# skhu101/TDNN-F_NAS

Hardware: AMD Instinct MI355X
Metric: LF-MMI training frames/sec per node (SWBD 7q TDNN-F) (higher is better)
Workload: dtype f32

## Files before the change

### tdnn-f_nas_amd/csrc/abi_tdnn.hip

```cpp
#include <dlfcn.h>
#include <stdlib.h>
#include <string.h>

#include <string>

#include "common.h"
#include "gemm_f32.h"
#include "planes_gemm.h"

namespace tdnnf {

static thread_local std::string g_last_error;

void set_error(const char *fmt, ...) {
  char buf[1024];
  va_list ap;
  va_start(ap, fmt);
  vsnprintf(buf, sizeof(buf), fmt, ap);
  va_end(ap);
  g_last_error = buf;
}
int hip_status(hipError_t e, const char *what) {
  set_error("HIP error %d (%s) in %s", (int)e, hipGetErrorString(e), what);
  return TDNNF_EHIP;
}

Options &options() {
  static Options o;
  return o;
}

namespace {
typedef int (*roctx_push_t)(const char *);
typedef int (*roctx_pop_t)();
roctx_push_t g_roctx_push = nullptr;
roctx_pop_t g_roctx_pop = nullptr;
bool roctx_ready() {
  static const bool ok = [] {
    const char *e = getenv("TDNNF_ROCTX");
    if (e && atoi(e) == 0) return false;
    for (const char *lib : {"librocprofiler-sdk-roctx.so", "librocprofiler-sdk-roctx.so.1", "libroctx64.so", "libroctx64.so.4"}) {
      void *h = dlopen(lib, RTLD_NOW | RTLD_GLOBAL);
      if (!h) continue;
      g_roctx_push = (roctx_push_t)dlsym(h, "roctxRangePushA");
      g_roctx_pop = (roctx_pop_t)dlsym(h, "roctxRangePop");
      if (g_roctx_push && g_roctx_pop) return true;
    }
    return false;
  }();
  return ok;
}
}
TraceRange::TraceRange(const char *name) : on(roctx_ready()) {
  if (on) g_roctx_push(name);
}
TraceRange::~TraceRange() {
  if (on) g_roctx_pop();
}

bool tdnn_rows_ok(const tdnnf_tdnn_indexes *ix, int rows_in, int N) {
  if (!ix || ix->num_offsets < 1 || ix->num_offsets > TDNNF_MAX_OFFSETS || ix->row_stride < 1) return false;
  for (int i = 0; i < ix->num_offsets; i++) {
    const long long need = (long long)ix->row_offsets[i] + (long long)ix->row_stride * N - (ix->row_stride - 1);
    if (ix->row_offsets[i] < 0 || (N > 0 && rows_in < need)) return false;
  }
  return true;
}

}

using namespace tdnnf;

extern "C" {

const char *tdnnf_last_error(void) { return g_last_error.c_str(); }
int tdnnf_abi_version(void) { return 1; }

static int *option_slot(const char *name) {
  Options &o = options();
  if (!name) return nullptr;
  const struct { const char *n; int *p; } table[] = {{"ng_grouped", &o.ng_grouped}, {"ng_fuse", &o.ng_fuse}, {"ng_early_in", &o.ng_early_in},
                                                     {"wgrad_stream", &o.wgrad_stream}, {"gemm_ring", &o.gemm_ring}, {"planes", &o.planes}, {"den_split", &o.den_split}, {"phase_events", &o.phase_events}, {"wgrad_lag", &o.wgrad_lag}, {"ng_bk", &o.ng_bk}, {"ng_valu", &o.ng_valu}, {"ng_pform", &o.ng_pform}, {"planes_group", &o.planes_group}, {"xent_behind_den", &o.xent_behind_den}, {"ng_early_fork", &o.ng_early_fork}, {"ng_diag_skip", &o.ng_diag_skip}, {"wgrad_small", &o.wgrad_small}, {"splitk_per_cu", &o.splitk_per_cu}, {"gemm_alt_taps", &o.gemm_alt_taps}, {"reverse_passes", &o.reverse_passes}, {"splitk_partial_round", &o.splitk_partial_round}, {"wgrad_on_caller", &o.wgrad_on_caller}, {"den_mw_test_abort", &o.den_mw_test_abort}, {"planes_check_bound", &o.planes_check_bound}, {"den_gamma_pairs", &o.den_gamma_pairs}, {"num_form", &o.num_form}, {"align_form", &o.align_form}, {"align_checkpoint", &o.align_checkpoint}, {"align_path_checkpoint", &o.align_path_checkpoint}, {"num_frontier_cap", &o.num_frontier_cap}, {"gemm_arith_test", &o.gemm_arith_test}};
  for (auto &e : table)
    if (strcmp(e.n, name) == 0) return e.p;
  return nullptr;
}
int tdnnf_set_option(const char *name, int value) {
  int *p = option_slot(name);
  TDNNF_REQUIRE(p, "set_option: unknown option '%s' (ng_grouped, ng_fuse, ng_early_in, wgrad_stream, gemm_ring, planes, den_split, align_checkpoint, align_path_checkpoint)", name ? name : "(null)");
  *p = value;
  return TDNNF_OK;
}
int tdnnf_get_option(const char *name, int *value) {
  int *p = option_slot(name);
  TDNNF_REQUIRE(p && value, "get_option: unknown option '%s'", name ? name : "(null)");
  *value = *p;
  return TDNNF_OK;
}

}

namespace tdnnf {
int tdnn_propagate_impl(const tdnnf_tdnn_indexes *ix, const tdnnf_mat *in, const float *W, int ldw, int Do, int Di,
                        const float *bias, const float *eff_coef, int init_mode, int relu, tdnnf_mat *out, tdnnf_stream stream,
                        float *colstats, int *colstats_rows) {
  TDNNF_REQUIRE(mat_ok(in) && mat_ok(out) && W, "tdnn_propagate: bad matrices");
  TDNNF_REQUIRE(Do > 0 && Di > 0 && in->cols == Di && out->cols == Do, "tdnn_propagate: dims: in.cols=%d Di=%d out.cols=%d Do=%d",
                in ? in->cols : -1, Di, out ? out->cols : -1, Do);
  TDNNF_REQUIRE(tdnn_rows_ok(ix, in->rows, out->rows), "tdnn_propagate: input has too few rows for the time offsets");
  TDNNF_REQUIRE(ldw >= ix->num_offsets * Di, "tdnn_propagate: ldw < K*Di");
  TDNNF_REQUIRE(init_mode >= 0 && init_mode <= 2 && (init_mode != 1 || bias), "tdnn_propagate: init_mode 1 needs a bias");
  RowsGemmArgs a;
  memset(&a, 0, sizeof(a));
  a.A = in->data;
  a.lda = (long long)in->stride * ix->row_stride;
  a.B = W;
  a.ldb = ldw;
  a.C = out->data;
  a.ldc = out->stride;
  a.M = out->rows;
  a.N = Do;
  a.bias = bias;
  a.coef = eff_coef;
  a.init_mode = init_mode;
  a.relu = relu;
  a.colstats = colstats;
  a.colstats_rows = colstats_rows;
  a.nseg = ix->num_offsets;
  for (int i = 0; i < a.nseg; i++) {
    a.seg[i].a_off = (long long)ix->row_offsets[i] * in->stride;
    a.seg[i].b_off = (long long)i * Di;
    a.seg[i].klen = Di;
    a.seg[i].m_lo = 0;
    a.seg[i].m_hi = out->rows;
  }
  TDNNF_HIP(rows_gemm(a, true, (hipStream_t)stream));
  return TDNNF_OK;
}
}

extern "C" {

int tdnnf_tdnn_propagate(const tdnnf_tdnn_indexes *ix, const tdnnf_mat *in, const float *W, int ldw, int Do, int Di,
                         const float *bias, const float *eff_coef, int init_mode, tdnnf_mat *out, tdnnf_stream stream) {
  return tdnn_propagate_impl(ix, in, W, ldw, Do, Di, bias, eff_coef, init_mode, 0, out, stream);
}

}

namespace tdnnf {
int tdnn_backprop_data_impl(const tdnnf_tdnn_indexes *ix, const tdnnf_mat *out_deriv, const float *W, int ldw, int Do,
                            int Di, const float *eff_coef, int overwrite, const tdnnf_mat *add, float add_scale, int add_lo,
                            tdnnf_mat *in_deriv, tdnnf_stream stream) {
  TDNNF_REQUIRE(mat_ok(in_deriv) && mat_ok(out_deriv) && W, "tdnn_backprop_data: bad matrices");
  TDNNF_REQUIRE(Do > 0 && Di > 0 && in_deriv->cols == Di && out_deriv->cols == Do, "tdnn_backprop_data: bad dims");
  TDNNF_REQUIRE(tdnn_rows_ok(ix, in_deriv->rows, out_deriv->rows), "tdnn_backprop_data: in_deriv has too few rows for the time offsets");
  TDNNF_REQUIRE(ldw >= ix->num_offsets * Di, "tdnn_backprop_data: ldw < K*Di");
  const int rho = ix->row_stride, N = out_deriv->rows, K = ix->num_offsets;
  if (N == 0) return TDNNF_OK;
  for (int cls = 0; cls < rho; cls++) {
    RowsGemmArgs a;
    memset(&a, 0, sizeof(a));
    float cf_dummy = 0;
    (void)cf_dummy;
    int nseg = 0, u_max = 0;
// ... 171 lines not shown
```

### tdnn-f_nas_amd/csrc/common.h

```cpp
#pragma once
#include <hip/hip_runtime.h>
#include <stdarg.h>
#include <stdio.h>

#include "tdnnf_hip.h"

namespace tdnnf {

struct MatView {
  float *data;
  int rows, cols, stride;
};
inline MatView view(const tdnnf_mat *m) { return MatView{m->data, m->rows, m->cols, m->stride}; }

void set_error(const char *fmt, ...);
int hip_status(hipError_t e, const char *what);

inline bool mat_ok(const tdnnf_mat *m) {
  return m && m->rows >= 0 && m->cols >= 0 && m->stride >= m->cols && (m->data || m->rows * m->cols == 0);
}
inline bool same_dim(const tdnnf_mat *a, const tdnnf_mat *b) { return a->rows == b->rows && a->cols == b->cols; }

inline bool vec4_ok(const MatView &m) {
  return (reinterpret_cast<uintptr_t>(m.data) & 15) == 0 && m.stride % 4 == 0 && m.cols % 4 == 0;
}

#define TDNNF_REQUIRE(cond, ...)            \
  do {                                      \
    if (!(cond)) {                          \
      ::tdnnf::set_error(__VA_ARGS__);      \
      return TDNNF_EINVAL;                  \
    }                                       \
  } while (0)

#define TDNNF_HIP(expr)                                         \
  do {                                                          \
    hipError_t e__ = (expr);                                    \
    if (e__ != hipSuccess) return ::tdnnf::hip_status(e__, #expr); \
  } while (0)

#define TDNNF_LAUNCH_CHECK() TDNNF_HIP(hipGetLastError())

struct Options {
  int ng_grouped = 1;
  int ng_fuse = 1;
  int ng_early_in = 1;
  int wgrad_stream = -1;
  int gemm_ring = 1;
  int planes = 1;
  int den_mw_test_abort = 0;
  int planes_group = 1;
  int planes_check_bound = 0;
  int wgrad_lag = 3;
  int wgrad_on_caller = 0;
  int splitk_partial_round = 1;
  int reverse_passes = 0;
  int gemm_alt_taps = 1;
  int splitk_per_cu = 2;
  int wgrad_small = 0;
  int ng_bk = 0;
  int ng_early_fork = 1;
  int xent_behind_den = -1;
  int ng_pform = 1;
  int ng_valu = 0;
  int ng_diag_skip = 0;
  int phase_events = 0;
  int den_split = -1;
  int num_form = 0;
  int gemm_arith_test = 0;
  int num_frontier_cap = 0;
  int align_form = 0;
  int align_checkpoint = 0;
  int align_path_checkpoint = 0;
  int den_gamma_pairs = 0;
};
Options &options();

struct TraceRange {
  explicit TraceRange(const char *name);
  ~TraceRange();
  bool on;
};

__host__ __device__ inline float floor_keep_nan(float x, float f) { return x < f ? f : x; }

inline int grid_for(long long work, int block, int cap = 2048) {
  long long g = (work + block - 1) / block;
  if (g > cap) g = cap;
  if (g < 1) g = 1;
  return (int)g;
}
#ifdef __HIPCC__
template <class T>
struct as_given { typedef T type; };
template <class... P>
__attribute__((visibility("hidden"))) inline hipError_t launch_vec_or_scalar(bool vec, int rows, int cols, void (*k4)(P...), void (*k1)(P...), hipStream_t s, typename as_given<P>::type... args) {
  const long long work = (long long)rows * (vec ? cols / 4 : cols);
  void (*k)(P...) = vec ? k4 : k1;
  hipLaunchKernelGGL(k, dim3(grid_for(work, 256)), dim3(256), 0, s, args...);
  return hipGetLastError();
}
#endif

inline unsigned long long tdnnf_decision(unsigned long long step, unsigned long long k) {
  unsigned long long z = step * 0x9E3779B97F4A7C15ULL + k * 0xBF58476D1CE4E5B9ULL + 0x94D049BB133111EBULL;
  z = (z ^ (z >> 30)) * 0xBF58476D1CE4E5B9ULL;
  z = (z ^ (z >> 27)) * 0x94D049BB133111EBULL;
  return (z ^ (z >> 31)) >> 8;
}

bool log_softmax_propagate_with_aux(const tdnnf_mat *in, tdnnf_mat *out, tdnnf_mat *aux, float aux_scale, hipStream_t s);
float chain_supervision_weight(const tdnnf_supervision *sp);
size_t chain_split_region_bytes(const tdnnf_den_graph *g, int B, int T);
int chain_den(const tdnnf_den_graph *g, const tdnnf_supervision *sp, const tdnnf_mat *y, float leaky, tdnnf_mat *deriv, void *ws, hipStream_t s,
              bool beside_other_work = false, hipStream_t caller_aux = nullptr, hipEvent_t ev_recursions = nullptr, bool *ev_recorded = nullptr);
int chain_num_recursion(const tdnnf_supervision *sp, const tdnnf_den_graph *g, const tdnnf_mat *y, void *ws, hipStream_t s);
int chain_num_xent(const tdnnf_den_graph *g, const tdnnf_supervision *sp, const tdnnf_mat *y, const tdnnf_mat *xent_output, float xent_regularize,
                   tdnnf_mat *xent_deriv, void *ws, hipStream_t s, bool xent_deriv_initialised = false);
int chain_num(const tdnnf_den_graph *g, const tdnnf_supervision *sp, const tdnnf_mat *y, const tdnnf_mat *xent_output,
              float xent_regularize, tdnnf_mat *xent_deriv, void *ws, hipStream_t s, bool xent_deriv_initialised = false);
int chain_finish(const tdnnf_den_graph *g, const tdnnf_supervision *sp, const tdnnf_mat *y, float l2_regularize, double *results,
                 tdnnf_mat *deriv, tdnnf_mat *xent_deriv, void *ws, hipStream_t s);
int chain_objf_den(const tdnnf_den_graph *g, const tdnnf_supervision *sp, const tdnnf_mat *y, float leaky, void *ws, hipStream_t s);
int chain_objf_num_recursion(const tdnnf_supervision *sp, const tdnnf_den_graph *g, const tdnnf_mat *y, void *ws, hipStream_t s);
int chain_objf_num_xent(const tdnnf_den_graph *g, const tdnnf_supervision *sp, const tdnnf_mat *y, const tdnnf_mat *xent_output, void *ws, hipStream_t s);
int chain_objf_finish(const tdnnf_den_graph *g, const tdnnf_supervision *sp, const tdnnf_mat *y, float l2_regularize, double *results, void *ws, hipStream_t s);

bool tdnn_rows_ok(const tdnnf_tdnn_indexes *ix, int rows_in, int N);
int tdnn_propagate_impl(const tdnnf_tdnn_indexes *ix, const tdnnf_mat *in, const float *W, int ldw, int Do, int Di,
                        const float *bias, const float *eff_coef, int init_mode, int relu, tdnnf_mat *out, tdnnf_stream stream,
                        float *colstats = nullptr, int *colstats_rows = nullptr);
int tdnn_update_simple_impl(const tdnnf_tdnn_indexes *ix, const tdnnf_mat *in_value, const tdnnf_mat *out_deriv, int Do, int Di,
                            const float *eff_coef, float lr, float *W_acc, int ldw, float *bias_acc, void *ws, size_t ws_bytes,
                            const int *active_dev, int max_active, tdnnf_stream stream, bool overwrite = false);
int tdnn_backprop_data_impl(const tdnnf_tdnn_indexes *ix, const tdnnf_mat *out_deriv, const float *W, int ldw, int Do, int Di,
                            const float *eff_coef, int overwrite, const tdnnf_mat *add, float add_scale, int add_lo,
                            tdnnf_mat *in_deriv, tdnnf_stream stream);

}
// ... 1 lines not shown
```

### tdnn-f_nas_amd/csrc/fused.hip

```cpp
#include <algorithm>

#include "batchnorm.h"
#include "device.h"
#include "ew_dev.h"
#include "fused.h"
#include "gemm_f32.h"
#include "launch_forms.h"
#include "planes_gemm.h"

namespace tdnnf {
namespace {

__device__ __forceinline__ void store_planes4(const PlanesSink &pk, float ps, long long ra, int c, const float (&v)[4]) {
  typedef _Float16 h4 __attribute__((ext_vector_type(4)));
  h4 hi, lo;
#pragma unroll
  for (int j = 0; j < 4; j++) {
    const float w = v[j] * ps;
    hi[j] = (_Float16)w;
    lo[j] = (_Float16)(w - (float)hi[j]);
  }
  const int kb = c >> 4, k = c & 15, half = (k >> 3) ^ (int)((ra >> 3) & 1);
  _Float16 *dst = reinterpret_cast<_Float16 *>(pk.P) + (((long long)kb * 2) * pk.R + ra) * 16 + half * 8 + (k & 7);
  *reinterpret_cast<h4 *>(dst) = hi;
  *reinterpret_cast<h4 *>(dst + pk.R * 16) = lo;
}

template <int VEC, bool PLANES>
__global__ __launch_bounds__(256) void bn_apply_bypass_kernel(MatView x, const float *mean, const float *scale, int D, int period,
                                                              MatView prev, float bypass, MatView out, const float *mask, int B, PlanesSink pk, int rev) {
  const int cv = x.cols / VEC;
  const float ps = PLANES ? pk.rec[0] : 1.0f;
  const int ncb = PLANES ? cv / 8 : 1;
  const long long total = PLANES ? (long long)((x.rows + 7) / 8) * 8 * cv : (long long)x.rows * cv;
  for (long long e0 = blockIdx.x * 256LL + threadIdx.x; e0 < total; e0 += gridDim.x * 256LL) {
    const long long e = rev ? total - 1 - e0 : e0;
    int r, c;
    if (PLANES) {
      const long long blk = e >> 6;
      r = (int)(blk / ncb) * 8 + (int)((e >> 3) & 7);
      c = ((int)(blk % ncb) * 8 + (int)(e & 7)) * VEC;
      if (r >= x.rows) continue;
    } else {
      r = (int)(e / cv);
      c = (int)(e % cv) * VEC;
    }
    const int cd = c % period;
    if (cd >= D) continue;
    float xv[4], pv[4] = {0, 0, 0, 0}, o[4];
    ld(x.data + (long long)r * x.stride + c, xv, VEC == 4);
    if (prev.data) ld(prev.data + (long long)r * prev.stride + c, pv, VEC == 4);
    const float *mk = mask ? mask + (long long)(x.cols > D ? c / period : r % B) * D + cd : nullptr;
    float mu[4], sc[4], mv[4] = {1.f, 1.f, 1.f, 1.f};
    ld(mean + cd, mu, VEC == 4);
    ld(scale + cd, sc, VEC == 4);
    if (mk) ld(mk, mv, VEC == 4);
#pragma unroll
    for (int j = 0; j < VEC; j++) o[j] = (xv[j] - mu[j]) * sc[j] * mv[j] + bypass * pv[j];
    st(out.data + (long long)r * out.stride + c, o, VEC == 4);
    if constexpr (PLANES && VEC == 4) store_planes4(pk, ps, r, c, o);
  }
}

template <int VEC, bool RELU_STATS>
__global__ __launch_bounds__(256) void bn_relu_bwd_reduce_kernel(MatView x, MatView dz, const float *mean, const float *scale,
                                                                 int rows_per_chunk, int chunks, float *partial, const float *mask, int B) {
  __shared__ float red[5][4][64 * 4 + 4];
  const int tc = threadIdx.x & 63, tr = threadIdx.x >> 6;
  const int col = (blockIdx.x * 64 + tc) * VEC;
  const int r0 = blockIdx.y * rows_per_chunk, r1 = min(x.rows, r0 + rows_per_chunk);
  float s[5][4] = {};
  if (col < x.cols) {
    float mu[4], sc[4];
#pragma unroll
    for (int j = 0; j < VEC; j++) {
      mu[j] = mean[col + j];
      sc[j] = scale[col + j];
    }
    for (int r = r0 + tr; r < r1; r += 4) {
      float xv[4], dv[4];
      ld(x.data + (long long)r * x.stride + col, xv, VEC == 4);
      ld(dz.data + (long long)r * dz.stride + col, dv, VEC == 4);
      if (mask) {
        const float *mk = mask + (long long)(r % B) * x.cols + col;
#pragma unroll
        for (int j = 0; j < VEC; j++) dv[j] *= mk[j];
      }
#pragma unroll
      for (int j = 0; j < VEC; j++) {
        const float z = (xv[j] - mu[j]) * sc[j];
        s[0][j] += z * dv[j];
        s[1][j] += dv[j];
        s[2][j] += dv[j] * dv[j];
        if (RELU_STATS) {
          s[3][j] += xv[j];
          s[4][j] += xv[j] > 0.f ? 1.f : 0.f;
        }
      }
    }
  }
  constexpr int NQ = RELU_STATS ? 5 : 3;
#pragma unroll
  for (int q = 0; q < NQ; q++)
#pragma unroll
    for (int j = 0; j < VEC; j++) red[q][tr][tc * VEC + j] = s[q][j];
  __syncthreads();
  if (tr == 0 && col < x.cols) {
#pragma unroll
    for (int q = 0; q < NQ; q++)
#pragma unroll
      for (int j = 0; j < VEC; j++) {
        const int k = tc * VEC + j;
        partial[((long long)q * chunks + blockIdx.y) * x.cols + col + j] = (red[q][0][k] + red[q][1][k]) + (red[q][2][k] + red[q][3][k]);
      }
  }
}

__global__ __launch_bounds__(kFinThreads) void bn_relu_bwd_finalize_kernel(const float *partial, int chunks, int D, int N, float target_rms,
                                                                           float *memo, double *relu_stats, int test_mode, double *oderiv,
                                                                           double *sums_out = nullptr, const double *sums_in = nullptr, int N_local = 0,
                                                                           double *fro2 = nullptr, float repair_abs = 0.f) {
  __shared__ double red[5 * kFinLanes * (kFinCols + 1)];
  const int d = blockIdx.x * kFinCols + (threadIdx.x & (kFinCols - 1));
  double q[5];
  const int nq = relu_stats ? 5 : 3;
  if (!sums_in) finalize_sums<5, double>(partial, chunks, chunks, D, nq, q, red);
  if (sums_out) {
    if (threadIdx.x < kFinCols && d < D)
      for (int k = 0; k < nq; k++) sums_out[(size_t)k * D + d] = q[k];
    return;
  }
  if (relu_stats && blockIdx.x == 0 && threadIdx.x == 0) relu_stats[0] += (double)(sums_in ? N_local : N);
  if (oderiv && blockIdx.x == 0 && threadIdx.x == 0) oderiv[0] += (double)N;
  double bound = 0;
  if (threadIdx.x < kFinCols && d < D) {
    if (sums_in)
      for (int k = 0; k < nq; k++) q[k] = sums_in[(size_t)k * D + d];
    const float coeff = -1.0f / (target_rms * target_rms * N);
    const float sc = memo[2 * D + d];
    const float vdm = test_mode ? 0.f : (float)(coeff * q[0]) * sc;
    memo[3 * D + d] = vdm;
    memo[4 * D + d] = test_mode ? 0.f : (float)(-q[1] / N);
    if (relu_stats) {
      relu_stats[1 + d] += q[3];
      relu_stats[1 + D + d] += q[4];
    }
    if (oderiv || fro2) {
      const double sc2 = (double)sc * sc;
      double v = sc2 * (test_mode ? q[2] : q[2] - q[1] * q[1] / N);
      if (!test_mode) {
        const double var = (double)memo[D + d] - (double)memo[d] * memo[d];
        v += 2.0 * vdm * sc * q[0] + (double)vdm * vdm * (double)N * (var > 0 ? var : 0.0) * sc2;
      }
      if (oderiv) oderiv[1 + d] += v > 0 ? v : 0.0;
      const double nr = sqrt(v > 0 ? v : 0.0) * 1.0001 + sqrt((double)N) * repair_abs;
      bound = nr * nr;
    }
  }
  if (fro2 && threadIdx.x < 64) {
    for (int o = 16; o > 0; o >>= 1) bound += __shfl_xor(bound, o, 32);
    if (threadIdx.x == 0) fro2[blockIdx.x] = bound;
  }
}

template <int VEC, bool PLANES>
__global__ __launch_bounds__(256) void bn_relu_bwd_apply_kernel(MatView x, MatView dz, const float *memo, int D,
                                                                const double *repair_stats, float self_repair_scale,
                                                                int rows_per_chunk, int chunks, MatView d_aff, float *partial, const float *mask, int B,
                                                                PlanesSink pk, int pk_lead, int rev) {
  const float pks = PLANES ? pk.rec[0] : 1.0f;
  __shared__ float red[4][64 * 4 + 4];
  const int tc = threadIdx.x & 63, tr = threadIdx.x >> 6;
  const int col = (blockIdx.x * 64 + tc) * VEC;
  const int chunk = rev ? (int)gridDim.y - 1 - (int)blockIdx.y : (int)blockIdx.y;
  const int r0 = chunk * rows_per_chunk, r1 = min(x.rows, r0 + rows_per_chunk);
  float s[4] = {0, 0, 0, 0};
  if (col < x.cols) {
    float mu[4], sc[4], vdm[4], tmp[4], rep[4];
#pragma unroll
    for (int j = 0; j < VEC; j++) {
      mu[j] = memo[col + j];
// ... 156 lines not shown
      const int idx = t + 256 * j, n = idx >> 3, kk = (idx & 7) * 4;
      *reinterpret_cast<float4 *>(Bs + n * LD + kk) = wv[j];
    }
    if (k0 + BK < D) request(k0 + BK);
#pragma unroll
    for (int i = 0; i < 4; i++) {
      const int r = r0 + rr + 32 * i;
      if (FULL || r < x.rows) {
        st(d_aff.data + (long long)r * d_aff.stride + col, o[i], true);
        if constexpr (PLANES) store_planes4(pk, pks, (long long)pk_lead + r, col, o[i]);
      }
    }
#pragma unroll
    for (int j = 0; j < 4; j++) {
      float v = cs[j];
      v += __shfl_xor(v, 8, 64);
      v += __shfl_xor(v, 16, 64);
      v += __shfl_xor(v, 32, 64);
      if (lane < 8) colred[wave][lane * 4 + j] = v;
    }
    __syncthreads();
    {
      const float *as = As + (wave * 32 + li) * LD + lh * 4;
      const float *bs = Bs + li * LD + lh * 4;
#pragma unroll
      for (int kg = 0; kg < BK / 8; kg++) {
        const float4 a = *reinterpret_cast<const float4 *>(as + kg * 8);
#pragma unroll
        for (int j = 0; j < NT; j++) {
          const float4 b = *reinterpret_cast<const float4 *>(bs + j * 32 * LD + kg * 8);
          acc[j] = __builtin_amdgcn_mfma_f32_32x32x2f32(a.x, b.x, acc[j], 0, 0, 0);
          acc[j] = __builtin_amdgcn_mfma_f32_32x32x2f32(a.y, b.y, acc[j], 0, 0, 0);
          acc[j] = __builtin_amdgcn_mfma_f32_32x32x2f32(a.z, b.z, acc[j], 0, 0, 0);
          acc[j] = __builtin_amdgcn_mfma_f32_32x32x2f32(a.w, b.w, acc[j], 0, 0, 0);
        }
      }
    }
    if (t < BK) partial[(long long)blk * D + k0 + t] = (colred[0][t] + colred[1][t]) + (colred[2][t] + colred[3][t]);
    __syncthreads();
  }
#pragma unroll
  for (int j = 0; j < NT; j++) {
    const int n = j * 32 + li;
#pragma unroll
    for (int e = 0; e < 16; e++) {
      const int r = r0 + wave * 32 + (e & 3) + 8 * (e >> 2) + 4 * lh;
      if (n < ng.Rp && r < x.rows) ng.H[(long long)r * ng.Rp + n] = acc[j][e];
    }
  }
  double v = ssq;
  for (int o = 32; o > 0; o >>= 1) v += __shfl_xor(v, o, 64);
  if (lane == 0) red[wave] = v;
  __syncthreads();
  if (t == 0) ng.part[blk] = (red[0] + red[1]) + (red[2] + red[3]);
  if (blk == 0)
    for (int i = gridDim.x + t; i < ng.part_cap; i += 256) ng.part[i] = 0.0;
}

template <int NT, bool MASK, bool PLANES>
__global__ __launch_bounds__(256) void bn_relu_bwd_apply_ng_kernel(MatView x, MatView dz, const float *memo, int D, const double *repair_stats,
                                                                   float self_repair_scale, MatView d_aff, float *partial, const float *mask, int B,
                                                                   NgFuse ng, PlanesSink pk, int pk_lead, int rev) {
  const int blk = rev ? (int)gridDim.x - 1 - (int)blockIdx.x : (int)blockIdx.x;
  if (blk * 128 + 128 <= x.rows)
    bn_relu_bwd_apply_ng_body<NT, MASK, true, PLANES>(x, dz, memo, D, repair_stats, self_repair_scale, d_aff, partial, mask, B, ng, pk, pk_lead, blk);
  else bn_relu_bwd_apply_ng_body<NT, MASK, false, PLANES>(x, dz, memo, D, repair_stats, self_repair_scale, d_aff, partial, mask, B, ng, pk, pk_lead, blk);
}

}

hipError_t bn_apply_bypass(MatView x, const float *memo, int D, int period, MatView prev, float bypass, MatView out, hipStream_t s, const float *mask, int B,
                           const PlanesSink *planes) {
  if (x.rows == 0) return hipSuccess;
  const bool vec = vec4_ok(x) && vec4_ok(out) && (!prev.data || vec4_ok(prev)) && D % 4 == 0 && (reinterpret_cast<uintptr_t>(memo) & 15) == 0 &&
                   (!mask || (reinterpret_cast<uintptr_t>(mask) & 15) == 0);
  const long long work = (long long)x.rows * (vec ? x.cols / 4 : x.cols);
  if (planes && !(vec && x.cols == D && D % 32 == 0 && planes->P && planes->rec)) return hipErrorInvalidValue;
  ProfHbmRange prof(4, 4.0 * x.rows * x.cols * ((prev.data ? 3.0 : 2.0) + (planes ? 1.0 : 0.0)), s);
  const PlanesSink none{nullptr, 0, nullptr};
  const int rev = vec && !planes ? options().reverse_passes & 1 : 0;
  count_fused(kFusedBypassFirst + (planes ? kFusedPlanes : vec ? kFusedVec4 : kFusedScalar) * 8 + (x.cols > D ? kFusedFlagSuper : 0) + (mask ? kFusedFlagMask : 0) +
              (rev ? kFusedFlagRev : 0));
  if (planes) hipLaunchKernelGGL((bn_apply_bypass_kernel<4, true>), dim3(grid_for((long long)((x.rows + 7) / 8) * 8 * (x.cols / 4), 256)), dim3(256), 0, s, x, memo, memo + 2 * D, D, period, prev, bypass, out, mask, B, *planes, 0);
  else if (vec) hipLaunchKernelGGL((bn_apply_bypass_kernel<4, false>), dim3(grid_for(work, 256)), dim3(256), 0, s, x, memo, memo + 2 * D, D, period, prev, bypass, out, mask, B, none, rev);
  else hipLaunchKernelGGL((bn_apply_bypass_kernel<1, false>), dim3(grid_for(work, 256)), dim3(256), 0, s, x, memo, memo + 2 * D, D, period, prev, bypass, out, mask, B, none, 0);
  return hipGetLastError();
}

bool bn_relu_bwd_ng_ok(MatView x, MatView dz, MatView d_aff, int Rp) {
  return vec4_ok(x) && vec4_ok(dz) && vec4_ok(d_aff) && x.cols % 32 == 0 && Rp >= 1 && Rp <= 96 && x.rows >= 1;
}

bool bn_relu_bwd_ng_pays(int rows) {
  const int slots = 2 * device_cus();
  const int blocks = (rows + 127) / 128, rounds = (blocks + slots - 1) / slots;
  return 4 * blocks >= 3 * rounds * slots;
}

size_t bn_relu_bwd_workspace_bytes(int rows, int cols) {
  ColReducePlan p = colreduce_plan(rows, cols);
  const size_t blocks128 = ((size_t)rows + 127) / 128;
  return sizeof(float) * (5 * (size_t)p.chunks + std::max((size_t)p.chunks, blocks128)) * cols + 64;
}

hipError_t bn_relu_bwd(MatView x, MatView dz, float *memo, float target_rms, bool bn_test_mode, double *relu_stats, bool store_relu_stats,
                       bool self_repair, float self_repair_scale, MatView d_aff, float *bias_acc, float bias_scale,
                       void *ws, size_t ws_bytes, hipStream_t s, const float *mask, int B, const NgFuse *ng, double *oderiv_stats, const BwdPlanes *planes) {
  if (x.rows == 0) return hipSuccess;
  if (ws_bytes < bn_relu_bwd_workspace_bytes(x.rows, x.cols)) return hipErrorInvalidValue;
  if (ng && (!bn_relu_bwd_ng_ok(x, dz, d_aff, ng->Rp) || (reinterpret_cast<uintptr_t>(memo) & 15) || (reinterpret_cast<uintptr_t>(ng->W) & 15) || ng->ldw % 4))
    return hipErrorInvalidValue;
  const int D = x.cols;
  ProfHbmRange prof(5, 4.0 * x.rows * x.cols * 5.0, s);
  ColReducePlan pl = colreduce_plan(x.rows, D);
  const bool vec = vec4_ok(x) && vec4_ok(dz) && vec4_ok(d_aff);
  const int per = vec ? 256 : 64;
  dim3 grid((D + per - 1) / per, pl.chunks), block(256);
  float *partial = (float *)ws;
  float *bias_partial = partial + 5 * (size_t)pl.chunks * D;
  count_fused(kFusedReduceFirst + (vec ? 0 : 2) + (store_relu_stats ? 1 : 0));
  count_fused(bn_test_mode ? kFusedFinalizeTest : kFusedFinalizeTrain);
  if (self_repair) count_fused(kFusedRepair);
  if (store_relu_stats) {
    if (vec) hipLaunchKernelGGL((bn_relu_bwd_reduce_kernel<4, true>), grid, block, 0, s, x, dz, memo, memo + 2 * D, pl.rows_per_chunk, pl.chunks, partial, mask, B);
    else hipLaunchKernelGGL((bn_relu_bwd_reduce_kernel<1, true>), grid, block, 0, s, x, dz, memo, memo + 2 * D, pl.rows_per_chunk, pl.chunks, partial, mask, B);
  } else {
    if (vec) hipLaunchKernelGGL((bn_relu_bwd_reduce_kernel<4, false>), grid, block, 0, s, x, dz, memo, memo + 2 * D, pl.rows_per_chunk, pl.chunks, partial, mask, B);
    else hipLaunchKernelGGL((bn_relu_bwd_reduce_kernel<1, false>), grid, block, 0, s, x, dz, memo, memo + 2 * D, pl.rows_per_chunk, pl.chunks, partial, mask, B);
  }
  double *fro2 = fro_bound_buf();
  if (fro2 && fro_bound_blocks()) *fro_bound_blocks() = (int)finalize_grid(D);
  const float repair_abs = self_repair ? 2.0f * fabsf(self_repair_scale) : 0.f;
  hipError_t fe = bn_finalize_synced(bn_test_mode ? nullptr : bn_sync_current(), 3, D, x.rows, s, [&](double *sums_out, const double *sums_in, int N) {
    hipLaunchKernelGGL(bn_relu_bwd_finalize_kernel, dim3(finalize_grid(D)), dim3(kFinThreads), 0, s, partial, pl.chunks, D, N, target_rms, memo,
                       store_relu_stats ? relu_stats : (double *)nullptr, bn_test_mode ? 1 : 0, oderiv_stats, sums_out, sums_in, x.rows, fro2, repair_abs);
  });
  if (fe != hipSuccess) return fe;
  const double *rep = self_repair ? relu_stats : nullptr;
  PlanesSink pk{nullptr, 0, nullptr};
  int pk_lead = 0;
  if (planes && planes->P) {
    if (!(fro2 && vec && x.cols % 16 == 0)) return hipErrorInvalidValue;
    hipError_t e = planes_scale_bound(fro2, (int)finalize_grid(D), (double)x.rows * D, 1.0f, 0.0f, nullptr, planes->rec, s);
    if (e != hipSuccess) return e;
    pk = PlanesSink{planes->P, planes->R, planes->rec};
    pk_lead = planes->lead;
  }
  const int rev = (options().reverse_passes >> 1) & 1;
  if (ng) {
    const int blocks = (x.rows + 127) / 128;
    count_fused(kFusedNgFirst + (ng->Rp <= 32 ? 0 : ng->Rp <= 64 ? 1 : 2) * 8 + (mask ? kFusedNgFlagMask : 0) + (pk.P ? kFusedNgFlagPlanes : 0) +
                (rev ? kFusedNgFlagRev : 0));
    count_fused(x.rows % 128 ? kFusedNgPartialBlock : kFusedNgFullBlocks);
#define APPLY_NG(NT)                                                                                                                                     \
  do {                                                                                                                                               \
    if (pk.P && mask) hipLaunchKernelGGL((bn_relu_bwd_apply_ng_kernel<NT, true, true>), dim3(blocks), block, 0, s, x, dz, memo, D, rep, self_repair_scale, d_aff, bias_partial, mask, B, *ng, pk, pk_lead, rev); \
    else if (pk.P) hipLaunchKernelGGL((bn_relu_bwd_apply_ng_kernel<NT, false, true>), dim3(blocks), block, 0, s, x, dz, memo, D, rep, self_repair_scale, d_aff, bias_partial, mask, B, *ng, pk, pk_lead, rev); \
    else if (mask) hipLaunchKernelGGL((bn_relu_bwd_apply_ng_kernel<NT, true, false>), dim3(blocks), block, 0, s, x, dz, memo, D, rep, self_repair_scale, d_aff, bias_partial, mask, B, *ng, pk, pk_lead, rev); \
    else hipLaunchKernelGGL((bn_relu_bwd_apply_ng_kernel<NT, false, false>), dim3(blocks), block, 0, s, x, dz, memo, D, rep, self_repair_scale, d_aff, bias_partial, mask, B, *ng, pk, pk_lead, rev);    \
  } while (0)
    if (ng->Rp <= 32) APPLY_NG(1);
    else if (ng->Rp <= 64) APPLY_NG(2);
    else APPLY_NG(3);
#undef APPLY_NG
    return bias_acc ? colsum_finalize(bias_partial, blocks, D, bias_scale, bias_acc, s) : hipGetLastError();
  }
  count_fused(kFusedApplyFirst + (pk.P ? kFusedPlanes : vec ? kFusedVec4 : kFusedScalar) * 4 + (mask ? 1 : 0) + (rev ? 2 : 0));
  {
    const int last = x.rows - (pl.chunks - 1) * pl.rows_per_chunk;
    bool unrolled = false, tail = false;
    for (int n : {pl.chunks > 1 ? pl.rows_per_chunk : last, last})
      for (int tr = 0; tr < 4 && tr < n; tr++) {
        const int m = (n - tr + 3) / 4;
        unrolled |= m >= 4;
        tail |= m % 4 != 0;
      }
    if (unrolled) count_fused(kFusedApplyUnrolled);
    if (tail) count_fused(kFusedApplyTail);
    if (pl.chunks > 1 && last < pl.rows_per_chunk) count_fused(kFusedApplyShortChunk);
  }
  if (pk.P) hipLaunchKernelGGL((bn_relu_bwd_apply_kernel<4, true>), grid, block, 0, s, x, dz, memo, D, rep, self_repair_scale, pl.rows_per_chunk, pl.chunks, d_aff, bias_partial, mask, B, pk, pk_lead, rev);
  else if (vec) hipLaunchKernelGGL((bn_relu_bwd_apply_kernel<4, false>), grid, block, 0, s, x, dz, memo, D, rep, self_repair_scale, pl.rows_per_chunk, pl.chunks, d_aff, bias_partial, mask, B, pk, pk_lead, rev);
  else hipLaunchKernelGGL((bn_relu_bwd_apply_kernel<1, false>), grid, block, 0, s, x, dz, memo, D, rep, self_repair_scale, pl.rows_per_chunk, pl.chunks, d_aff, bias_partial, mask, B, pk, pk_lead, rev);
  return bias_acc ? colsum_finalize(bias_partial, pl.chunks, D, bias_scale, bias_acc, s) : hipGetLastError();
}

}
```

### tdnn-f_nas_amd/csrc/launch_forms.h

```cpp
#pragma once
#include <atomic>

namespace tdnnf {

enum RowsForm {
  kFormPlain,
  kFormRing,
  kFormSplitK,
  kFormPartialS2,
  kFormPartialS8 = kFormPartialS2 + 6,
  kFormMainSplitTail,
  kFormMainPlainTail,
  kFormSumsqPlain,
  kFormSumsqSplitK,
  kFormPost,
  kFormGrouped,
  kRowsForms
};
constexpr int kRowsTiles = 9, kRowsAriths = 3;

template <int WM, int WN, int TM, int TN, int BK>
constexpr int rows_tile_index() {
  constexpr int BM = WM * TM * 32, BN = WN * TN * 32;
  constexpr int t = (BM == 128 && BN == 32 && BK == 32) ? 0 : (BM == 128 && BN == 32 && BK == 64) ? 1 : (BM == 128 && BN == 64 && BK == 32) ? 2
                  : (BM == 128 && BN == 96 && BK == 16) ? 3 : (BM == 128 && BN == 96 && BK == 32) ? 4 : (BM == 128 && BN == 160 && BK == 16) ? 5
                  : (BM == 64 && BN == 128 && BK == 16) ? 6 : (BM == 128 && BN == 128 && BK == 16) ? 7 : (BM == 128 && BN == 128 && BK == 32) ? 8 : -1;
  static_assert(t >= 0, "a rows GEMM tile without a counter: add it here and to kRowsTileNames (launch_forms.hip)");
  return t;
}
constexpr int rows_form_index(int tile, int arith, int form) { return (tile * kRowsAriths + arith) * kRowsForms + form; }

enum {
  kPlanesPlain = kRowsTiles * kRowsAriths * kRowsForms,
  kPlanesMainSplitTail,
  kPlanesMainPlainTail,
  kWgradFirst,
  kWgradPlanes = kWgradFirst + 5 * kRowsAriths,
  kWgradLastSlabs,
  kRowsLastSlices,
  kRowsVec4Launches,
  kRowsScalarLaunches,
  kPlanesAltChunked,
  kLaunchFormCounters
};

std::atomic<long long> *launch_form_counters();
inline void count_form(int index) { launch_form_counters()[index].fetch_add(1, std::memory_order_relaxed); }
inline void note_rows_slices(int ksplit) { launch_form_counters()[kRowsLastSlices].store(ksplit, std::memory_order_relaxed); }
inline void note_wgrad_slabs(int splits) { launch_form_counters()[kWgradLastSlabs].store(splits, std::memory_order_relaxed); }

enum { kFusedVec4, kFusedScalar, kFusedPlanes, kFusedKinds };
constexpr int kFusedFlagSuper = 1, kFusedFlagMask = 2, kFusedFlagRev = 4;
constexpr int kFusedNgFlagMask = 1, kFusedNgFlagPlanes = 2, kFusedNgFlagRev = 4;
enum FusedForm {
  kFusedBypassFirst,
  kFusedReduceFirst = kFusedBypassFirst + kFusedKinds * 8,
  kFusedFinalizeTrain = kFusedReduceFirst + 4,
  kFusedFinalizeTest,
  kFusedApplyFirst,
  kFusedApplyUnrolled = kFusedApplyFirst + kFusedKinds * 4,
  kFusedApplyTail,
  kFusedApplyShortChunk,
  kFusedNgFirst,
  kFusedNgPartialBlock = kFusedNgFirst + 3 * 8,
  kFusedNgFullBlocks,
  kFusedRepair,
  kFusedFormCounters
};
std::atomic<long long> *fused_form_counters();
inline void count_fused(int index) { fused_form_counters()[index].fetch_add(1, std::memory_order_relaxed); }

}
```

### tdnn-f_nas_amd/csrc/launch_forms.hip

```cpp
#include "launch_forms.h"

#include <stdio.h>

#include "common.h"

namespace tdnnf {

std::atomic<long long> *launch_form_counters() {
  static std::atomic<long long> counters[kLaunchFormCounters];
  return counters;
}

std::atomic<long long> *fused_form_counters() {
  static std::atomic<long long> counters[kFusedFormCounters];
  return counters;
}

namespace {
const char *const kFusedKindNames[kFusedKinds] = {"vec4", "scalar", "planes"};
const char *const kRowsTileNames[kRowsTiles] = {"128x32k32", "128x32k64", "128x64k32", "128x96k16", "128x96k32", "128x160k16", "64x128k16", "128x128k16", "128x128k32"};
const char *const kArithNames[kRowsAriths] = {"f32", "bf16x3", "bf16x6"};
const char *const kRowsFormNames[kRowsForms] = {"plain", "ring", "splitk", "partial_s2", "partial_s3", "partial_s4", "partial_s5", "partial_s6", "partial_s7", "partial_s8",
                                                "main_split_tail", "main_plain_tail", "sumsq_plain", "sumsq_splitk", "post", "grouped"};
const char *const kWgradTileNames[5] = {"128x128", "160x128", "128x160", "32x128", "64x64"};
}

}

using namespace tdnnf;

extern "C" {

const char *tdnnf_gemm_launch_form_name(int index) {
  static thread_local char buf[64];
  if (index < 0 || index >= kLaunchFormCounters) return nullptr;
  if (index < kPlanesPlain) {
    const int form = index % kRowsForms, arith = (index / kRowsForms) % kRowsAriths, tile = index / (kRowsForms * kRowsAriths);
    snprintf(buf, sizeof(buf), "rows.%s.%s.%s", kRowsTileNames[tile], kArithNames[arith], kRowsFormNames[form]);
  } else if (index == kPlanesPlain) {
    snprintf(buf, sizeof(buf), "planes.plain");
  } else if (index == kPlanesMainSplitTail) {
    snprintf(buf, sizeof(buf), "planes.main_split_tail");
  } else if (index == kPlanesMainPlainTail) {
    snprintf(buf, sizeof(buf), "planes.main_plain_tail");
  } else if (index < kWgradPlanes) {
    const int i = index - kWgradFirst;
    snprintf(buf, sizeof(buf), "wgrad.%s.%s", kWgradTileNames[i / kRowsAriths], kArithNames[i % kRowsAriths]);
  } else if (index == kWgradPlanes) {
    snprintf(buf, sizeof(buf), "wgrad.planes");
  } else if (index == kWgradLastSlabs) {
    snprintf(buf, sizeof(buf), "wgrad.last_slabs");
  } else if (index == kRowsLastSlices) {
    snprintf(buf, sizeof(buf), "rows.last_slices");
  } else if (index == kRowsVec4Launches) {
    snprintf(buf, sizeof(buf), "rows.launches_vec4");
  } else if (index == kRowsScalarLaunches) {
    snprintf(buf, sizeof(buf), "rows.launches_scalar");
  } else {
    snprintf(buf, sizeof(buf), "planes.alt_chunked");
  }
  return buf;
}

int tdnnf_gemm_launch_forms(long long *counts, int capacity, int reset) {
  std::atomic<long long> *c = launch_form_counters();
  for (int i = 0; i < kLaunchFormCounters; i++) {
    if (counts && i < capacity) counts[i] = c[i].load(std::memory_order_relaxed);
    if (reset) c[i].store(0, std::memory_order_relaxed);
  }
  return kLaunchFormCounters;
}

const char *tdnnf_fused_launch_form_name(int index) {
  static thread_local char buf[64];
  if (index < 0 || index >= kFusedFormCounters) return nullptr;
  if (index < kFusedReduceFirst) {
    const int i = index - kFusedBypassFirst, f = i % 8;
    snprintf(buf, sizeof(buf), "apply_bypass.%s%s%s%s", kFusedKindNames[i / 8], f & kFusedFlagSuper ? ".super" : "", f & kFusedFlagMask ? ".mask" : "",
             f & kFusedFlagRev ? ".rev" : "");
  } else if (index < kFusedFinalizeTrain) {
    const int i = index - kFusedReduceFirst;
    snprintf(buf, sizeof(buf), "bwd.reduce.%s.%s", i & 2 ? "scalar" : "vec4", i & 1 ? "stats" : "nostats");
  } else if (index == kFusedFinalizeTrain) {
    snprintf(buf, sizeof(buf), "bwd.finalize.train");
  } else if (index == kFusedFinalizeTest) {
    snprintf(buf, sizeof(buf), "bwd.finalize.test");
  } else if (index < kFusedApplyUnrolled) {
    const int i = index - kFusedApplyFirst, f = i % 4;
    snprintf(buf, sizeof(buf), "bwd.apply.%s%s%s", kFusedKindNames[i / 4], f & 1 ? ".mask" : "", f & 2 ? ".rev" : "");
  } else if (index == kFusedApplyUnrolled) {
    snprintf(buf, sizeof(buf), "bwd.apply.rows_unrolled");
  } else if (index == kFusedApplyTail) {
    snprintf(buf, sizeof(buf), "bwd.apply.rows_tail");
  } else if (index == kFusedApplyShortChunk) {
    snprintf(buf, sizeof(buf), "bwd.apply.short_last_chunk");
  } else if (index < kFusedNgPartialBlock) {
    const int i = index - kFusedNgFirst, f = i % 8;
    snprintf(buf, sizeof(buf), "bwd.apply_ng.nt%d%s%s%s", i / 8 + 1, f & kFusedNgFlagMask ? ".mask" : "", f & kFusedNgFlagPlanes ? ".planes" : "",
             f & kFusedNgFlagRev ? ".rev" : "");
  } else if (index == kFusedNgPartialBlock) {
    snprintf(buf, sizeof(buf), "bwd.apply_ng.partial_block");
  } else if (index == kFusedNgFullBlocks) {
    snprintf(buf, sizeof(buf), "bwd.apply_ng.full_blocks");
  } else {
    snprintf(buf, sizeof(buf), "bwd.repair");
  }
  return buf;
}

int tdnnf_fused_launch_forms(long long *counts, int capacity, int reset) {
  std::atomic<long long> *c = fused_form_counters();
  for (int i = 0; i < kFusedFormCounters; i++) {
    if (counts && i < capacity) counts[i] = c[i].load(std::memory_order_relaxed);
    if (reset) c[i].store(0, std::memory_order_relaxed);
  }
  return kFusedFormCounters;
}

}
```

Baseline: 1.631 million.

## Add strip-mined bypass apply and 4-row-unrolled BN backward reduce kernels

Adds a new option, sweeps_form (default 1), that routes the vec4 BN-apply-bypass path to a strip kernel. In that kernel each thread walks a column strip over a chunk of rows, with the per-column mean and scale loaded once, four row loads issued before use, and the mask index stepped incrementally. A second bit (off by default) selects a 128-thread reduce kernel with 4-way unrolled row loads for the backward statistics. The aim is better memory-level parallelism and less per-element index arithmetic in these bandwidth-bound elementwise sweeps, at the cost of more register use and extra launch variants.

```diff
diff --git a/tdnn-f_nas_amd/csrc/abi_tdnn.hip b/tdnn-f_nas_amd/csrc/abi_tdnn.hip
--- a/tdnn-f_nas_amd/csrc/abi_tdnn.hip
+++ b/tdnn-f_nas_amd/csrc/abi_tdnn.hip
@@ -80,7 +80,7 @@
   Options &o = options();
   if (!name) return nullptr;
   const struct { const char *n; int *p; } table[] = {{"ng_grouped", &o.ng_grouped}, {"ng_fuse", &o.ng_fuse}, {"ng_early_in", &o.ng_early_in},
-                                                     {"wgrad_stream", &o.wgrad_stream}, {"gemm_ring", &o.gemm_ring}, {"planes", &o.planes}, {"den_split", &o.den_split}, {"phase_events", &o.phase_events}, {"wgrad_lag", &o.wgrad_lag}, {"ng_bk", &o.ng_bk}, {"ng_valu", &o.ng_valu}, {"ng_pform", &o.ng_pform}, {"planes_group", &o.planes_group}, {"xent_behind_den", &o.xent_behind_den}, {"ng_early_fork", &o.ng_early_fork}, {"ng_diag_skip", &o.ng_diag_skip}, {"wgrad_small", &o.wgrad_small}, {"splitk_per_cu", &o.splitk_per_cu}, {"gemm_alt_taps", &o.gemm_alt_taps}, {"reverse_passes", &o.reverse_passes}, {"splitk_partial_round", &o.splitk_partial_round}, {"wgrad_on_caller", &o.wgrad_on_caller}, {"den_mw_test_abort", &o.den_mw_test_abort}, {"planes_check_bound", &o.planes_check_bound}, {"den_gamma_pairs", &o.den_gamma_pairs}, {"num_form", &o.num_form}, {"align_form", &o.align_form}, {"align_checkpoint", &o.align_checkpoint}, {"align_path_checkpoint", &o.align_path_checkpoint}, {"num_frontier_cap", &o.num_frontier_cap}, {"gemm_arith_test", &o.gemm_arith_test}};
+                                                     {"wgrad_stream", &o.wgrad_stream}, {"gemm_ring", &o.gemm_ring}, {"planes", &o.planes}, {"den_split", &o.den_split}, {"phase_events", &o.phase_events}, {"wgrad_lag", &o.wgrad_lag}, {"ng_bk", &o.ng_bk}, {"ng_valu", &o.ng_valu}, {"ng_pform", &o.ng_pform}, {"planes_group", &o.planes_group}, {"xent_behind_den", &o.xent_behind_den}, {"ng_early_fork", &o.ng_early_fork}, {"ng_diag_skip", &o.ng_diag_skip}, {"wgrad_small", &o.wgrad_small}, {"splitk_per_cu", &o.splitk_per_cu}, {"gemm_alt_taps", &o.gemm_alt_taps}, {"reverse_passes", &o.reverse_passes}, {"sweeps_form", &o.sweeps_form}, {"splitk_partial_round", &o.splitk_partial_round}, {"wgrad_on_caller", &o.wgrad_on_caller}, {"den_mw_test_abort", &o.den_mw_test_abort}, {"planes_check_bound", &o.planes_check_bound}, {"den_gamma_pairs", &o.den_gamma_pairs}, {"num_form", &o.num_form}, {"align_form", &o.align_form}, {"align_checkpoint", &o.align_checkpoint}, {"align_path_checkpoint", &o.align_path_checkpoint}, {"num_frontier_cap", &o.num_frontier_cap}, {"gemm_arith_test", &o.gemm_arith_test}};
   for (auto &e : table)
     if (strcmp(e.n, name) == 0) return e.p;
   return nullptr;
diff --git a/tdnn-f_nas_amd/csrc/common.h b/tdnn-f_nas_amd/csrc/common.h
--- a/tdnn-f_nas_amd/csrc/common.h
+++ b/tdnn-f_nas_amd/csrc/common.h
@@ -55,6 +55,7 @@
   int wgrad_on_caller = 0;
   int splitk_partial_round = 1;
   int reverse_passes = 0;
+  int sweeps_form = 1;
   int gemm_alt_taps = 1;
   int splitk_per_cu = 2;
   int wgrad_small = 0;
diff --git a/tdnn-f_nas_amd/csrc/fused.hip b/tdnn-f_nas_amd/csrc/fused.hip
--- a/tdnn-f_nas_amd/csrc/fused.hip
+++ b/tdnn-f_nas_amd/csrc/fused.hip
@@ -62,6 +62,85 @@
   }
 }
 
+template <int VEC>
+__device__ __forceinline__ void pin_requested(float (&v)[4]) {
+  if (VEC == 4) {
+    typedef float f4 __attribute__((ext_vector_type(4)));
+    f4 t = {v[0], v[1], v[2], v[3]};
+    asm volatile("" : "+v"(t) : : "memory");
+    v[0] = t[0]; v[1] = t[1]; v[2] = t[2]; v[3] = t[3];
+  } else {
+    asm volatile("" : "+v"(v[0]) : : "memory");
+  }
+}
+
+template <bool PREV, int MASKMODE>
+__global__ __launch_bounds__(256) void bn_apply_bypass_strip_kernel(MatView x, const float *mean, const float *scale, int D, int period, MatView prev,
+                                                                    float bypass, MatView out, const float *mask, int B, int rows_per_chunk, int rev) {
+  const int tc = threadIdx.x & 63, tr = threadIdx.x >> 6;
+  const int c = (blockIdx.x * 64 + tc) * 4;
+  if (c >= x.cols) return;
+  const int cd = c % period;
+  if (cd >= D) return;
+  const int chunk = rev ? (int)gridDim.y - 1 - (int)blockIdx.y : (int)blockIdx.y;
+  const int r0 = chunk * rows_per_chunk, r1 = min(x.rows, r0 + rows_per_chunk);
+  int m = r1 - r0 > tr ? (r1 - r0 - tr + 3) / 4 : 0;
+  float mu[4], sc[4], mv[4] = {1.f, 1.f, 1.f, 1.f};
+  const float zero[4] = {0.f, 0.f, 0.f, 0.f};
+  ld(mean + cd, mu, true);
+  ld(scale + cd, sc, true);
+  if (MASKMODE == 2) ld(mask + (long long)(c / period) * D + cd, mv, true);
+  const int dr = rev ? -4 : 4;
+  int r = rev ? r1 - 1 - tr : r0 + tr;
+  int rb = 0, b4 = 0;
+  if (MASKMODE == 1 && m > 0) {
+    rb = r % B;
+    b4 = 4 % B;
+  }
+  auto step_rb = [&]() {
+    if (rev) {
+      rb -= b4;
+      if (rb < 0) rb += B;
+    } else {
+      rb += b4;
+      if (rb >= B) rb -= B;
+    }
+  };
+  auto finish = [&](const float (&xv)[4], const float (&pv)[4], const float (&mw)[4], int rr) {
+    float o[4];
+#pragma unroll
+    for (int j = 0; j < 4; j++) o[j] = __builtin_fmaf(bypass, pv[j], (xv[j] - mu[j]) * sc[j] * mw[j]);
+    st(out.data + (long long)rr * out.stride + c, o, true);
+  };
+  for (; m >= 4; m -= 4, r += 4 * dr) {
+    float xv[4][4], pv[4][4], mw[4][4];
+#pragma unroll
+    for (int u = 0; u < 4; u++) {
+      const int ru = r + u * dr;
+      ld(x.data + (long long)ru * x.stride + c, xv[u], true);
+      if (PREV) ld(prev.data + (long long)ru * prev.stride + c, pv[u], true);
+      if (MASKMODE == 1) {
+        ld(mask + (long long)rb * D + cd, mw[u], true);
+        step_rb();
+      }
+    }
+#pragma unroll
+    for (int u = 0; u < 4; u++) pin_requested<4>(xv[u]);
+#pragma unroll
+    for (int u = 0; u < 4; u++) finish(xv[u], PREV ? pv[u] : zero, MASKMODE == 1 ? mw[u] : mv, r + u * dr);
+  }
+  for (; m > 0; m--, r += dr) {
+    float xv[4], pv[4], mw[4];
+    ld(x.data + (long long)r * x.stride + c, xv, true);
+    if (PREV) ld(prev.data + (long long)r * prev.stride + c, pv, true);
+    if (MASKMODE == 1) {
+      ld(mask + (long long)rb * D + cd, mw, true);
+      step_rb();
+    }
+    finish(xv, PREV ? pv : zero, MASKMODE == 1 ? mw : mv, r);
+  }
+}
+
 template <int VEC, bool RELU_STATS>
 __global__ __launch_bounds__(256) void bn_relu_bwd_reduce_kernel(MatView x, MatView dz, const float *mean, const float *scale,
                                                                  int rows_per_chunk, int chunks, float *partial, const float *mask, int B) {
@@ -97,6 +176,85 @@
           s[4][j] += xv[j] > 0.f ? 1.f : 0.f;
         }
       }
+    }
+  }
+  constexpr int NQ = RELU_STATS ? 5 : 3;
+#pragma unroll
+  for (int q = 0; q < NQ; q++)
+#pragma unroll
+    for (int j = 0; j < VEC; j++) red[q][tr][tc * VEC + j] = s[q][j];
+  __syncthreads();
+  if (tr == 0 && col < x.cols) {
+#pragma unroll
+    for (int q = 0; q < NQ; q++)
+#pragma unroll
+      for (int j = 0; j < VEC; j++) {
+        const int k = tc * VEC + j;
+        partial[((long long)q * chunks + blockIdx.y) * x.cols + col + j] = (red[q][0][k] + red[q][1][k]) + (red[q][2][k] + red[q][3][k]);
+      }
+  }
+}
+
+template <int VEC, bool RELU_STATS, bool MASK>
+__global__ __launch_bounds__(128) void bn_relu_bwd_reduce4_kernel(MatView x, MatView dz, const float *mean, const float *scale,
+                                                                  int rows_per_chunk, int chunks, float *partial, const float *mask, int B) {
+  __shared__ float red[5][4][32 * 4 + 4];
+  const int tc = threadIdx.x & 31, tr = threadIdx.x >> 5;
+  const int col = (blockIdx.x * 32 + tc) * VEC;
+  const int r0 = blockIdx.y * rows_per_chunk, r1 = min(x.rows, r0 + rows_per_chunk);
+  float s[5][4] = {};
+  if (col < x.cols) {
+    float mu[4], sc[4];
+#pragma unroll
+    for (int j = 0; j < VEC; j++) {
+      mu[j] = mean[col + j];
+      sc[j] = scale[col + j];
+    }
+    auto request = [&](int r, float (&xv)[4], float (&dv)[4], float (&mk)[4]) {
+      ld(x.data + (long long)r * x.stride + col, xv, VEC == 4);
+      ld(dz.data + (long long)r * dz.stride + col, dv, VEC == 4);
+      if (MASK) {
+        const float *mp = mask + (long long)(r % B) * x.cols + col;
+#pragma unroll
+        for (int j = 0; j < VEC; j++) mk[j] = mp[j];
+      }
+    };
+    constexpr bool kFma0 = VEC == 4, kFma2 = VEC == 4 || !RELU_STATS;
+    auto add_row = [&](const float (&xv)[4], float (&dv)[4], const float (&mk)[4]) {
+#pragma clang fp contract(off)
+      if (MASK) {
+#pragma unroll
+        for (int j = 0; j < VEC; j++) dv[j] *= mk[j];
+      }
+#pragma unroll
+      for (int j = 0; j < VEC; j++) {
+        const float z = (xv[j] - mu[j]) * sc[j];
+        s[0][j] = kFma0 ? __builtin_fmaf(z, dv[j], s[0][j]) : s[0][j] + z * dv[j];
+        s[1][j] += dv[j];
+        s[2][j] = kFma2 ? __builtin_fmaf(dv[j], dv[j], s[2][j]) : s[2][j] + dv[j] * dv[j];
+        if (RELU_STATS) {
+          s[3][j] += xv[j];
+          s[4][j] += xv[j] > 0.f ? 1.f : 0.f;
+        }
+      }
+    };
+    int r = r0 + tr;
+    for (; r + 12 < r1; r += 16) {
+      float xv[4][4], dv[4][4], mk[4][4];
+#pragma unroll
+      for (int u = 0; u < 4; u++) request(r + 4 * u, xv[u], dv[u], mk[u]);
+#pragma unroll
+      for (int u = 0; u < 4; u++) {
+        pin_requested<VEC>(xv[u]);
+        pin_requested<VEC>(dv[u]);
+      }
+#pragma unroll
+      for (int u = 0; u < 4; u++) add_row(xv[u], dv[u], mk[u]);
+    }
+    for (; r < r1; r += 4) {
+      float xv[4], dv[4], mk[4];
+      request(r, xv, dv, mk);
+      add_row(xv, dv, mk);
     }
   }
   constexpr int NQ = RELU_STATS ? 5 : 3;
@@ -419,7 +577,26 @@
   count_fused(kFusedBypassFirst + (planes ? kFusedPlanes : vec ? kFusedVec4 : kFusedScalar) * 8 + (x.cols > D ? kFusedFlagSuper : 0) + (mask ? kFusedFlagMask : 0) +
               (rev ? kFusedFlagRev : 0));
   if (planes) hipLaunchKernelGGL((bn_apply_bypass_kernel<4, true>), dim3(grid_for((long long)((x.rows + 7) / 8) * 8 * (x.cols / 4), 256)), dim3(256), 0, s, x, memo, memo + 2 * D, D, period, prev, bypass, out, mask, B, *planes, 0);
-  else if (vec) hipLaunchKernelGGL((bn_apply_bypass_kernel<4, false>), dim3(grid_for(work, 256)), dim3(256), 0, s, x, memo, memo + 2 * D, D, period, prev, bypass, out, mask, B, none, rev);
+  else if (vec && (options().sweeps_form & 1)) {
+    count_fused(kFusedForm1Bypass);
+    const int colblocks = (x.cols / 4 + 63) / 64;
+    const int chunks = std::max(1, std::min(std::max(1, 8 * device_cus() / colblocks), (x.rows + 15) / 16));
+    const int rows_per_chunk = (x.rows + chunks - 1) / chunks;
+    const dim3 grid(colblocks, (x.rows + rows_per_chunk - 1) / rows_per_chunk);
+    const int mode = !mask ? 0 : x.cols > D ? 2 : 1;
+#define BYPASS_STRIP(PREV, MODE) \
+  hipLaunchKernelGGL((bn_apply_bypass_strip_kernel<PREV, MODE>), grid, dim3(256), 0, s, x, memo, memo + 2 * D, D, period, prev, bypass, out, mask, B, rows_per_chunk, rev)
+    if (prev.data) {
+      if (mode == 0) BYPASS_STRIP(true, 0);
+      else if (mode == 1) BYPASS_STRIP(true, 1);
+      else BYPASS_STRIP(true, 2);
+    } else {
+      if (mode == 0) BYPASS_STRIP(false, 0);
+      else if (mode == 1) BYPASS_STRIP(false, 1);
+      else BYPASS_STRIP(false, 2);
+    }
+#undef BYPASS_STRIP
+  } else if (vec) hipLaunchKernelGGL((bn_apply_bypass_kernel<4, false>), dim3(grid_for(work, 256)), dim3(256), 0, s, x, memo, memo + 2 * D, D, period, prev, bypass, out, mask, B, none, rev);
   else hipLaunchKernelGGL((bn_apply_bypass_kernel<1, false>), dim3(grid_for(work, 256)), dim3(256), 0, s, x, memo, memo + 2 * D, D, period, prev, bypass, out, mask, B, none, 0);
   return hipGetLastError();
 }
@@ -458,7 +635,36 @@
   count_fused(kFusedReduceFirst + (vec ? 0 : 2) + (store_relu_stats ? 1 : 0));
   count_fused(bn_test_mode ? kFusedFinalizeTest : kFusedFinalizeTrain);
   if (self_repair) count_fused(kFusedRepair);
-  if (store_relu_stats) {
+  if (options().sweeps_form & 2) {
+    count_fused(kFusedForm1Reduce);
+    {
+      const int last = x.rows - (pl.chunks - 1) * pl.rows_per_chunk;
+      bool unrolled = false, tail = false;
+      for (int n : {pl.chunks > 1 ? pl.rows_per_chunk : last, last})
+        for (int tr = 0; tr < 4 && tr < n; tr++) {
+          const int m = (n - tr + 3) / 4;
+          unrolled |= m >= 4;
+          tail |= m % 4 != 0;
+        }
+      if (unrolled) count_fused(kFusedReduceUnrolled);
+      if (tail) count_fused(kFusedReduceTail);
+    }
+    const int per4 = vec ? 128 : 32;
+    const dim3 grid4((D + per4 - 1) / per4, pl.chunks), block4(128);
+#define REDUCE4(VEC, STATS)                                                                                                                              \
+  do {                                                                                                                                                   \
+    if (mask) hipLaunchKernelGGL((bn_relu_bwd_reduce4_kernel<VEC, STATS, true>), grid4, block4, 0, s, x, dz, memo, memo + 2 * D, pl.rows_per_chunk, pl.chunks, partial, mask, B); \
+    else hipLaunchKernelGGL((bn_relu_bwd_reduce4_kernel<VEC, STATS, false>), grid4, block4, 0, s, x, dz, memo, memo + 2 * D, pl.rows_per_chunk, pl.chunks, partial, mask, B);     \
+  } while (0)
+    if (store_relu_stats) {
+      if (vec) REDUCE4(4, true);
+      else REDUCE4(1, true);
+    } else {
+      if (vec) REDUCE4(4, false);
+      else REDUCE4(1, false);
+    }
+#undef REDUCE4
+  } else if (store_relu_stats) {
     if (vec) hipLaunchKernelGGL((bn_relu_bwd_reduce_kernel<4, true>), grid, block, 0, s, x, dz, memo, memo + 2 * D, pl.rows_per_chunk, pl.chunks, partial, mask, B);
     else hipLaunchKernelGGL((bn_relu_bwd_reduce_kernel<1, true>), grid, block, 0, s, x, dz, memo, memo + 2 * D, pl.rows_per_chunk, pl.chunks, partial, mask, B);
   } else {
diff --git a/tdnn-f_nas_amd/csrc/launch_forms.h b/tdnn-f_nas_amd/csrc/launch_forms.h
--- a/tdnn-f_nas_amd/csrc/launch_forms.h
+++ b/tdnn-f_nas_amd/csrc/launch_forms.h
@@ -65,6 +65,10 @@
   kFusedNgPartialBlock = kFusedNgFirst + 3 * 8,
   kFusedNgFullBlocks,
   kFusedRepair,
+  kFusedReduceUnrolled,
+  kFusedReduceTail,
+  kFusedForm1Reduce,
+  kFusedForm1Bypass,
   kFusedFormCounters
 };
 std::atomic<long long> *fused_form_counters();
diff --git a/tdnn-f_nas_amd/csrc/launch_forms.hip b/tdnn-f_nas_amd/csrc/launch_forms.hip
--- a/tdnn-f_nas_amd/csrc/launch_forms.hip
+++ b/tdnn-f_nas_amd/csrc/launch_forms.hip
@@ -102,8 +102,16 @@
     snprintf(buf, sizeof(buf), "bwd.apply_ng.partial_block");
   } else if (index == kFusedNgFullBlocks) {
     snprintf(buf, sizeof(buf), "bwd.apply_ng.full_blocks");
+  } else if (index == kFusedRepair) {
+    snprintf(buf, sizeof(buf), "bwd.repair");
+  } else if (index == kFusedReduceUnrolled) {
+    snprintf(buf, sizeof(buf), "bwd.reduce.rows_unrolled");
+  } else if (index == kFusedReduceTail) {
+    snprintf(buf, sizeof(buf), "bwd.reduce.rows_tail");
+  } else if (index == kFusedForm1Reduce) {
+    snprintf(buf, sizeof(buf), "sweeps_form.bwd.reduce");
   } else {
-    snprintf(buf, sizeof(buf), "bwd.repair");
+    snprintf(buf, sizeof(buf), "sweeps_form.apply_bypass");
   }
   return buf;
 }
```

Result: no change. 1.631 million, median of 2 (+0.0%).
